# IBM/DeepRest

Measured on AMD Instinct MI355X. Metric: training samples/sec, 256-endpoint 3-resource estimation model, higher is better.
Workload: dtype bf16; 1 GPU; model=deeprest-amd (attention encoder + call-graph + GRU decoders), endpoints=256, components=63, num_metrics=192, global_batch=2048, seq_len=60, parallelism=dp1

## Files before the change

deeprest_amd/csrc/bindings.cpp:

```cpp
#include <torch/extension.h>
#include <ATen/cuda/CUDAContext.h>
#include <c10/cuda/CUDAGuard.h>
#include <hip/hip_runtime.h>

#include <cmath>
#include <string>
#include <vector>

extern "C" {
void dr_dropout_add_ln_fwd(const void* branch, const void* residual, const float* w,
                           const float* b, const int64_t* seed, uint32_t thr,
                           float scale, void* r_out, void* normed, float* mean,
                           float* rstd, int64_t n_rows, int D, float eps,
                           int is_bf16, hipStream_t stream);
void dr_dropout_add_ln_bwd(const void* d_normed, const void* d_r_out,
                           const void* r_out, const float* w, const float* mean,
                           const float* rstd, const int64_t* seed, uint32_t thr,
                           float scale, void* d_res, void* d_branch,
                           float* dwdb_part, int n_blocks, int64_t n_rows, int D,
                           int is_bf16, hipStream_t stream);
void dr_pinball_fwd(const void* out, const float* labels, const float* quantiles,
                    int Q, int64_t N, float inv_count, float* loss, int is_bf16,
                    hipStream_t stream);
void dr_pinball_bwd(const void* out, const float* labels, const float* quantiles,
// ... 4 lines not shown
                           const float* quantiles, int Q, int64_t R, int M,
                           float* wsum, int* wcnt, float* loss, float* w,
                           int is_bf16, hipStream_t stream);
void dr_pinball_masked_bwd(const void* out, const float* labels,
                           const float* quantiles, int Q, int64_t R, int M,
                           const float* grad_loss, const float* w, void* dout,
                           int is_bf16, hipStream_t stream);
void dr_fused_adam(const int64_t* meta, int nt, int64_t total, float lr, float beta1,
                   float beta2, float eps, float weight_decay, int step,
                   hipStream_t stream);
void dr_fused_adam_dev(const int64_t* meta, int nt, int64_t total,
                       const float* lr_ptr, float beta1, float beta2, float eps,
                       float weight_decay, const int* step_ptr,
                       hipStream_t stream);
int dr_gru_fwd_fuses_heads(int B, int C);
int dr_gru_fwd(const void* xg, const void* gamma, const void* beta,
               const void* w_hh, const float* b_hh, const void* h0, void* h_all,
               void* saves, const void* wh_fwd, void* out, int O, int B, int TT,
               int C, int reverse, int save, int fp8, int is_bf16,
               hipStream_t stream);
int dr_gru_decode(const void* xg, const void* gamma, const void* beta,
                  const void* w_hh, const float* b_hh, const void* h0,
                  const void* wh_fwd, void* out, void* h_last, int B, int TT,
                  int C, int O, int reverse, int fp8, int is_bf16,
                  const int* lens, hipStream_t stream);
int dr_gru_bwd(const void* grad, const void* wh_img, int O, const void* w_img,
               const void* w_fwd, const void* xg, const void* gamma,
               const void* beta, const float* b_hh, const void* h0,
               const void* h_all, const void* saves, void* dpre, float* dh0,
               int B, int TT, int C, int reverse, int is_bf16,
               hipStream_t stream);
int dr_gru_reduce_fused_max_c();
int dr_gru_bwd_reduce(const void* dpre, const void* gamma, const void* xg,
                      void* dxg, float* dgamma, float* dbeta, void* gamma_pi,
                      void* xg_pi, int64_t BT, int C, int mode, int is_bf16,
                      hipStream_t stream);
void dr_mha_fwd(const void* q, const void* k, const void* v, void* o, float* lse,
                int64_t BH, int T_len, int D, float scale, int is_bf16,
                const int* kv_len, int n_heads, hipStream_t stream);
void dr_mha_bwd(const void* q, const void* k, const void* v, const void* o,
                const void* dout, const float* lse, float* dq, void* dk, void* dv,
                int64_t BH, int T_len, int D, float scale, int is_bf16,
                hipStream_t stream);
int dr_sanity_scores(const void* out, const float* measured, const float* base,
                     const float* y_min, const float* y_scale,
// ... 349 lines not shown
              "gru operand dtypes must match x_gates");
  TORCH_CHECK(xg.is_contiguous() && w_hh.is_contiguous() && h0.is_contiguous() &&
              gamma.is_contiguous() && beta.is_contiguous() && b_hh.is_contiguous());
  TORCH_CHECK(xg.numel() < (1LL << 31),
              "x_gates too large for 32-bit staging offsets");
}

static void check_wh_fwd(const at::Tensor& wh_fwd, int64_t O, int H) {
  TORCH_CHECK(O >= 1 && O <= 32, "the fused head phase needs 1 <= O <= 32, got ", O);
  TORCH_CHECK(wh_fwd.scalar_type() == at::kBFloat16 &&
                  wh_fwd.sizes() == at::IntArrayRef({32, H}) &&
                  wh_fwd.is_contiguous() && wh_fwd.is_cuda(),
              "wh_fwd must be the (32, H) bf16 head weight image");
}

bool gru_fwd_fuses_heads(int64_t B, int64_t C, bool save) {
  return save && dr_gru_fwd_fuses_heads((int)B, (int)C) != 0;
}

std::vector<at::Tensor> gru_seq_forward(at::Tensor xg, at::Tensor w_hh,
                                        at::Tensor b_hh, at::Tensor h0,
                                        at::Tensor gamma, at::Tensor beta,
                                        bool reverse, bool save, bool fp8,
                                        c10::optional<at::Tensor> wh_fwd,
                                        int64_t O) {
  TORCH_CHECK(!(fp8 && save), "fp8 GRU path is inference-only (no saves)");
  const at::cuda::CUDAGuard guard(xg.device());
  gru_forward_checks(xg, w_hh, b_hh, h0, gamma, beta);
  int B = (int)xg.size(0), TT = (int)xg.size(1);
  int C = (int)h0.size(1), H = (int)h0.size(2);
// ... 2 lines not shown
  const bool heads = wh_fwd.has_value();
  if (heads) {
    TORCH_CHECK(!fp8 && gru_fwd_fuses_heads(B, C, save),
                "gru forward: no in-kernel head phase at B=", B, " C=", C,
                " save=", save, " (ask gru_fwd_fuses_heads first)");
    check_wh_fwd(*wh_fwd, O, H);
    TORCH_CHECK((int64_t)B * TT * C * O < (1LL << 31),
                "head output too large for 32-bit store offsets");
  }
  auto h_all = at::empty({B, TT, C, H}, xg.options());
  auto saves = save ? at::empty({B, TT, C, 2 * H}, xg.options())
                    : at::empty({0}, xg.options());
  auto out = heads ? at::empty({B, TT, C, O}, xg.options())
                   : at::empty({0}, xg.options());
  auto w_gemm = gru_w_gemm(w_hh);
  gru_launch_check(
      dr_gru_fwd(xg.data_ptr(), gamma.data_ptr(), beta.data_ptr(),
                 w_gemm.data_ptr(), b_hh.data_ptr<float>(), h0.data_ptr(),
                 h_all.data_ptr(), save ? saves.data_ptr() : nullptr,
                 heads ? wh_fwd->data_ptr() : nullptr,
                 heads ? out.data_ptr() : nullptr, heads ? (int)O : 0, B, TT, C,
                 reverse ? 1 : 0, save ? 1 : 0, fp8 ? 1 : 0, is_bf16(xg),
                 cur_stream()),
      "gru forward");
  if (!heads) return {h_all, saves};
  return {h_all, saves, out};
}

std::vector<at::Tensor> gru_seq_decode(at::Tensor xg, at::Tensor w_hh,
                                       at::Tensor b_hh, at::Tensor h0,
                                       at::Tensor gamma, at::Tensor beta,
                                       at::Tensor wh_fwd, int64_t O, bool reverse,
                                       bool fp8,
                                       c10::optional<at::Tensor> lengths) {
  const at::cuda::CUDAGuard guard(xg.device());
  gru_forward_checks(xg, w_hh, b_hh, h0, gamma, beta);
  int B = (int)xg.size(0), TT = (int)xg.size(1);
  int C = (int)h0.size(1), H = (int)h0.size(2);
  check_wh_fwd(wh_fwd, O, H);
  TORCH_CHECK((int64_t)B * TT * C * O < (1LL << 31),
              "decode output too large for 32-bit store offsets");
  const int* lens = lengths_ptr(lengths, xg, B, "gru decode lengths");
  auto out = lens ? at::zeros({B, TT, C, O}, xg.options())
                  : at::empty({B, TT, C, O}, xg.options());
  auto h_last = at::empty({B, C, H}, xg.options());
  auto w_gemm = gru_w_gemm(w_hh);
  gru_launch_check(
      dr_gru_decode(xg.data_ptr(), gamma.data_ptr(), beta.data_ptr(),
                    w_gemm.data_ptr(), b_hh.data_ptr<float>(), h0.data_ptr(),
                    wh_fwd.data_ptr(), out.data_ptr(), h_last.data_ptr(), B, TT,
                    C, (int)O, reverse ? 1 : 0, fp8 ? 1 : 0, is_bf16(xg), lens,
                    cur_stream()),
      "gru decode");
  return {out, h_last};
}

static std::vector<at::Tensor> gru_backward_impl(
    at::Tensor grad_h, const at::Tensor* wh_img, at::Tensor w_img,
    at::Tensor w_fwd, at::Tensor xg, at::Tensor gamma, at::Tensor beta,
    at::Tensor b_hh, at::Tensor h0, at::Tensor h_all, at::Tensor saves,
    bool reverse) {
  const at::cuda::CUDAGuard guard(grad_h.device());
  TORCH_CHECK(grad_h.dim() == 4 && h_all.dim() == 4, "grad and h_all must be 4-D");
  int B = (int)h_all.size(0), TT = (int)h_all.size(1);
  int C = (int)h_all.size(2), H = (int)h_all.size(3);
  TORCH_CHECK(H == 128);
  TORCH_CHECK(grad_h.size(0) == B && grad_h.size(1) == TT && grad_h.size(2) == C,
// ... 26 lines not shown
  TORCH_CHECK(w_img.scalar_type() == at::kBFloat16 &&
                  w_img.sizes() == at::IntArrayRef({H, 3 * H}) &&
                  w_img.is_contiguous(),
              "w_img must be the (H, 3H) bf16 pi-permuted W image");
  TORCH_CHECK(w_fwd.scalar_type() == at::kBFloat16 &&
                  w_fwd.sizes() == at::IntArrayRef({3 * H, H}) &&
                  w_fwd.is_contiguous(),
              "w_fwd must be the (3H, H) bf16 weight image");
  TORCH_CHECK(b_hh.scalar_type() == at::kFloat && b_hh.is_contiguous());
  auto dt = grad_h.scalar_type();
  TORCH_CHECK(xg.scalar_type() == dt && gamma.scalar_type() == dt &&
              beta.scalar_type() == dt);
  TORCH_CHECK(grad_h.is_contiguous() && h_all.is_contiguous() && saves.is_contiguous());
  auto dpre = at::empty({B, TT, C, 4 * H}, grad_h.options());
  auto dh0 = at::empty({B, C, H}, grad_h.options().dtype(at::kFloat));
  gru_launch_check(
      dr_gru_bwd(grad_h.data_ptr(), wh_img ? wh_img->data_ptr() : nullptr, O,
                 w_img.data_ptr(), w_fwd.data_ptr(), xg.data_ptr(),
                 gamma.data_ptr(), beta.data_ptr(), b_hh.data_ptr<float>(),
                 h0.data_ptr(), h_all.data_ptr(), saves.data_ptr(),
                 dpre.data_ptr(), dh0.data_ptr<float>(), B, TT, C,
                 reverse ? 1 : 0, dt == at::kBFloat16, cur_stream()),
      "gru backward");
  return {dpre, dh0};
}

std::vector<at::Tensor> gru_seq_backward_kernel(at::Tensor grad_h, at::Tensor w_img,
                                                at::Tensor w_fwd, at::Tensor xg,
                                                at::Tensor gamma, at::Tensor beta,
                                                at::Tensor b_hh, at::Tensor h0,
                                                at::Tensor h_all, at::Tensor saves,
                                                bool reverse) {
  return gru_backward_impl(grad_h, nullptr, w_img, w_fwd, xg, gamma, beta, b_hh,
                           h0, h_all, saves, reverse);
}

std::vector<at::Tensor> gru_seq_backward_heads_kernel(
// ... 198 lines not shown
```

deeprest_amd/csrc/common.h:

```cpp
#pragma once

#include <hip/hip_runtime.h>
#include <hip/hip_bf16.h>
#include <hip/hip_fp8.h>
#include <stdint.h>
#include <algorithm>

#define DR_WAVE 64

namespace dr {

__device__ __forceinline__ float bf2f(uint16_t x) {
  union { uint32_t u; float f; } v;
  v.u = static_cast<uint32_t>(x) << 16;
  return v.f;
}

__device__ __forceinline__ uint16_t f2bf(float f) {
  __hip_bfloat16 b = __float2bfloat16(f);
  return *reinterpret_cast<uint16_t*>(&b);
}

__device__ __forceinline__ uint32_t f2bf2(float lo, float hi) {
  __hip_bfloat162 b2 = __float22bfloat162_rn(make_float2(lo, hi));
// ... 42 lines not shown
}

__device__ __forceinline__ float group16_sum(float v) {
#pragma unroll
  for (int off = 8; off > 0; off >>= 1) v += __shfl_xor(v, off, DR_WAVE);
  return v;
}

__device__ __forceinline__ float group16_max(float v) {
#pragma unroll
  for (int off = 8; off > 0; off >>= 1) v = fmaxf(v, __shfl_xor(v, off, DR_WAVE));
  return v;
}

__device__ __forceinline__ float sigmoidf_(float x) {
  return __fdividef(1.0f, 1.0f + __expf(-x));
}

__device__ __forceinline__ float tanhf_(float x) {
  float xc = fminf(fmaxf(x, -15.f), 15.f);
  float e = __expf(2.f * xc);
  return __fdividef(e - 1.f, e + 1.f);
}

using f32x4 = __attribute__((__vector_size__(4 * sizeof(float)))) float;
using bf16x8 = __attribute__((ext_vector_type(8))) __bf16;
using s16x8 = __attribute__((ext_vector_type(8))) short;

}
```

deeprest_amd/csrc/gru.hip:

```cpp
#include "common.h"

#include <type_traits>

namespace dr {

constexpr int H = 128;
constexpr int G3H = 384;
constexpr int G4H = 512;
constexpr int ROWS = 64;
constexpr int WAVES = 4;
constexpr int THREADS = WAVES * DR_WAVE;
constexpr int KT = H / 32;
constexpr int NT = G3H / 16;
constexpr int XG_SLOTS = 32;

constexpr int LDS_MAX = 163840;

template <bool FP8, int NSUB, bool HEADS>
struct FwdLds {
  static constexpr int ELT = FP8 ? 1 : 2;
  static constexpr int W = 0;
  static constexpr int WH = W + G3H * H * ELT;
  static constexpr int HM = WH + (HEADS ? 32 * H * 2 : 0);
  static constexpr int XG = HM + ROWS * NSUB * H * ELT;
// ... 62 lines not shown
template <typename T>
__device__ __forceinline__ void ld8(const T* src, float* v);
template <>
__device__ __forceinline__ void ld8<uint16_t>(const uint16_t* src, float* v) {
  uint4 raw = *reinterpret_cast<const uint4*>(src);
  const uint16_t* p = reinterpret_cast<const uint16_t*>(&raw);
#pragma unroll
  for (int e = 0; e < 8; ++e) v[e] = bf2f(p[e]);
}
template <>
__device__ __forceinline__ void ld8<float>(const float* src, float* v) {
  *reinterpret_cast<float4*>(v) = *reinterpret_cast<const float4*>(src);
  *reinterpret_cast<float4*>(v + 4) = *reinterpret_cast<const float4*>(src + 4);
}

template <typename T>
__device__ __forceinline__ void st_frag(T* dst, bf16x8 v);
template <>
__device__ __forceinline__ void st_frag<uint16_t>(uint16_t* dst, bf16x8 v) {
  *reinterpret_cast<uint4*>(dst) = *reinterpret_cast<const uint4*>(&v);
}
template <>
__device__ __forceinline__ void st_frag<float>(float* dst, bf16x8 v) {
  const uint16_t* p = reinterpret_cast<const uint16_t*>(&v);
#pragma unroll
  for (int e = 0; e < 8; ++e) dst[e] = bf2f(p[e]);
}

template <typename T>
__device__ __forceinline__ void ld_raw8(const T* src, uint16_t* out);
// ... 9 lines not shown
}

template <typename T>
__device__ __forceinline__ bf16x8 ld_frag(const T* src);
template <>
__device__ __forceinline__ bf16x8 ld_frag<uint16_t>(const uint16_t* src) {
  return *reinterpret_cast<const bf16x8*>(src);
}
template <>
__device__ __forceinline__ bf16x8 ld_frag<float>(const float* src) {
  uint16_t p[8];
#pragma unroll
  for (int e = 0; e < 8; ++e) p[e] = f2bf(src[e]);
  return *reinterpret_cast<bf16x8*>(p);
}

template <typename T, bool SAVE, bool FP8 = false, int NSUB = 1, bool HEADS = false,
          bool VARLEN = false>
__global__ __launch_bounds__(THREADS * NSUB) void gru_fwd_kernel(
    const T* __restrict__ xg,
    const T* __restrict__ gamma,
    const T* __restrict__ beta,
    const uint16_t* __restrict__ w_gemm,
    const float* __restrict__ b_hh,
    const T* __restrict__ h0,
    T* __restrict__ h_all,
    T* __restrict__ saves,
    int B, int TT, int C, int reverse,
    const uint16_t* __restrict__ wh_fwd,
    T* __restrict__ out,
    T* __restrict__ h_last,
    int O,
    const int* __restrict__ lens) {
  static_assert(HEADS || !VARLEN, "per-row lengths exist in the decode kernel only");
  static_assert(!(SAVE && (VARLEN || FP8)),
                "the saving kernels run full windows on bf16 GEMM tiles");
  extern __shared__ __attribute__((aligned(16))) char smem[];
  using L = FwdLds<FP8, NSUB, HEADS>;
  constexpr int BROWS = ROWS * NSUB;
  constexpr int BTHREADS = THREADS * NSUB;
  char* Wl = smem + L::W;
  char* WHl = smem + L::WH;
  char* Hl = smem + L::HM;
  char* XGl = smem + L::XG;
  constexpr bool GB_REGS = (NSUB == 1) && !(VARLEN && FP8);

  const int tid = threadIdx.x;
  const int wv = tid / DR_WAVE;
  const int lane = tid % DR_WAVE;
  const int64_t R = (int64_t)B * C;
  const int64_t r0 = (int64_t)blockIdx.x * BROWS;

  for (int id = tid; id < G3H * (H / 8); id += BTHREADS) {
    int j = id / (H / 8);
    int blk = id % (H / 8);
    bf16x8 v = *reinterpret_cast<const bf16x8*>(w_gemm + (int64_t)j * H + blk * 8);
    if constexpr (FP8) {
      const uint16_t* bv = reinterpret_cast<const uint16_t*>(&v);
      uint8_t q[8];
#pragma unroll
// ... 28 lines not shown
    b_of[i] = (int)(rr / C);
    comp_of[i] = (int)(rr % C);
  }
  int len_of[4];
  if constexpr (VARLEN) {
#pragma unroll
    for (int i = 0; i < 4; ++i) {
      len_of[i] = std::min(std::max(lens[b_of[i]], 1), TT);
    }
  }

  constexpr int GBN = GB_REGS ? 8 : 1;
  uint32_t gb[4][3][GBN];
  float bh[3][GBN];
  int gb_off[4];
#pragma unroll
  for (int i = 0; i < 4; ++i) gb_off[i] = comp_of[i] * G3H;
  if constexpr (GB_REGS) {
#pragma unroll
    for (int i = 0; i < 4; ++i) {
      const T* grow = gamma + gb_off[i];
      const T* brow = beta + gb_off[i];
#pragma unroll
      for (int g = 0; g < 3; ++g)
#pragma unroll
        for (int nt = 0; nt < 8; ++nt) {
          int col = g * H + nt * 16 + c_col;
          uint16_t gv = live[i] ? f2bf(ldf(grow + col)) : 0;
          uint16_t bv = live[i] ? f2bf(ldf(brow + col)) : 0;
          gb[i][g][nt] = ((uint32_t)bv << 16) | gv;
        }
    }
// ... 58 lines not shown
  const uint16_t* xg_rows[4];
#pragma unroll
  for (int i = 0; i < 4; ++i)
    xg_rows[i] =
        reinterpret_cast<const uint16_t*>(XGl) +
        (wv * WSLOTS + std::min(b_of[i] - b_wlo, WSLOTS - 1)) * G3H + c_col * 8;

  __syncthreads();

  int stage_toff = 0;
  int bc_toff = 0;
  const int stage_tstep = (reverse ? -1 : 1) * G3H;
  for (int step = 0; step < TT; ++step) {
    const int t_now = reverse ? (TT - 1 - step) : step;
    (void)t_now;
    bf16x8 afrag[KT];
    int64_t afrag8[KT];
#pragma unroll
    for (int kt = 0; kt < KT; ++kt) {
      if constexpr (FP8)
        afrag8[kt] = *reinterpret_cast<const int64_t*>(Hl + afrag_off[kt]);
      else
        afrag[kt] = lds_read8(Hl, afrag_off[kt]);
    }

#pragma unroll
    for (int u = 0; u < MAXCH; ++u) {
      if (u < n_stage) {
        const T* src = xg + stage_soff[u] + stage_toff;
        uint16_t* dst = reinterpret_cast<uint16_t*>(XGl) + stage_pi0[u];
// ... 12 lines not shown
#pragma unroll
      for (int kt = 0; kt < KT; ++kt) {
        int j = nt * 16 + c_col;
        int k0 = kt * 32 + (lane >> 4) * 8;
        if constexpr (FP8) {
          int64_t bfrag = *reinterpret_cast<const int64_t*>(Wl + swz8(j, k0));
          a = __builtin_amdgcn_mfma_f32_16x16x32_fp8_fp8(afrag8[kt], bfrag, a, 0, 0, 0);
        } else {
          bf16x8 bfrag = lds_read8(Wl, swz(j, k0));
          a = __builtin_amdgcn_mfma_f32_16x16x32_bf16(afrag[kt], bfrag, a, 0, 0, 0);
        }
      }
      acc[nt] = a;
    }

    const T* gm_v = gamma;
    const T* bt_v = beta;
    const float* bh_v = b_hh;
    if constexpr (!GB_REGS) asm volatile("" : "+v"(gm_v), "+v"(bt_v), "+v"(bh_v));
#pragma unroll
    for (int i = 0; i < 4; ++i) {
      const T* grow = gm_v + gb_off[i];
      const T* brow = bt_v + gb_off[i];
      float fr[8], fz[8], fn[8];
      bool active = true;
      if constexpr (VARLEN) active = t_now < len_of[i];
#pragma unroll
      for (int nt = 0; nt < 8; ++nt) {
        float xr = bf2f(xg_rows[i][nt]);
        float xz = bf2f(xg_rows[i][H + nt]);
        float xn = bf2f(xg_rows[i][2 * H + nt]);
        int col = nt * 16 + c_col;
        float gmr, gmz, gmn, btr, btz, btn, bhr, bhz, bhn;
        if constexpr (GB_REGS) {
          gmr = bf2f((uint16_t)gb[i][0][nt]); btr = bf2f((uint16_t)(gb[i][0][nt] >> 16));
          gmz = bf2f((uint16_t)gb[i][1][nt]); btz = bf2f((uint16_t)(gb[i][1][nt] >> 16));
          gmn = bf2f((uint16_t)gb[i][2][nt]); btn = bf2f((uint16_t)(gb[i][2][nt] >> 16));
          bhr = bh[0][nt]; bhz = bh[1][nt]; bhn = bh[2][nt];
        } else if constexpr (NSUB == 1) {
          gmr = bf2f(f2bf(ldf(grow + col))); btr = bf2f(f2bf(ldf(brow + col)));
          gmz = bf2f(f2bf(ldf(grow + H + col)));
          btz = bf2f(f2bf(ldf(brow + H + col)));
          gmn = bf2f(f2bf(ldf(grow + 2 * H + col)));
          btn = bf2f(f2bf(ldf(brow + 2 * H + col)));
          bhr = bh_v[col]; bhz = bh_v[H + col]; bhn = bh_v[2 * H + col];
        } else {
          gmr = ldf(grow + col); btr = ldf(brow + col);
          gmz = ldf(grow + H + col); btz = ldf(brow + H + col);
          gmn = ldf(grow + 2 * H + col); btn = ldf(brow + 2 * H + col);
          bhr = bh_v[col]; bhz = bh_v[H + col]; bhn = bh_v[2 * H + col];
        }
        float g_r, g_z, g_n;
        if constexpr (!GB_REGS && NSUB == 1) {
          g_r = __fmul_rn(xr, gmr) + btr;
          g_z = __fmul_rn(xz, gmz) + btz;
          g_n = __builtin_fmaf(xn, gmn, btn);
        } else {
          g_r = xr * gmr + btr;
          g_z = xz * gmz + btz;
          g_n = xn * gmn + btn;
        }
        float rp = sigmoidf_(acc[nt][i] + bhr + g_r);
        float zp = sigmoidf_(acc[nt + 8][i] + bhz + g_z);
        float hn = acc[nt + 16][i] + bhn;
        float nn = tanhf_(g_n + rp * hn);
        float hnew = (1.f - zp) * nn + zp * h[i][nt];
        if constexpr (VARLEN) hnew = active ? hnew : h[i][nt];
        h[i][nt] = hnew;
        if constexpr (FP8)
          *reinterpret_cast<uint8_t*>(Hl + swz8(row_of[i], col)) = f2fp8(hnew);
        else
          *reinterpret_cast<uint16_t*>(Hl + swz(row_of[i], col)) = f2bf(hnew);
        fr[nt] = rp; fz[nt] = zp; fn[nt] = nn; (void)fn;
      }
      if (SAVE && live[i]) {
        T* sv = saves + (int64_t)(bc[i] + bc_toff) * (2 * H) + c_col * 8;
        st8(sv, fr);
        st8(sv + H, fz);
      }
      __builtin_amdgcn_sched_barrier(0);
    }
    wave_lds_fence();

    if constexpr (HEADS) {
      bf16x8 hfrag[KT];
#pragma unroll
      for (int kt = 0; kt < KT; ++kt) {
        if constexpr (FP8) {
          uint64_t raw = *reinterpret_cast<const uint64_t*>(Hl + afrag_off[kt]);
          const uint8_t* q = reinterpret_cast<const uint8_t*>(&raw);
          uint16_t p[8];
#pragma unroll
          for (int e = 0; e < 8; ++e) {
            __hip_fp8_e4m3 x;
            x.__x = q[e];
// ... 206 lines not shown
        const int jl = nt * 16 + c_col;
#pragma unroll
        for (int kt = 0; kt < KT; ++kt) {
          bf16x8 bfrag;
          if constexpr (NSUB == 2)
            bfrag = lds_read8(wn_lds, swz(jl, kt * 32 + k0));
          else
            bfrag = *reinterpret_cast<const bf16x8*>(
                wfv + (int64_t)(2 * H + jl) * H + kt * 32 + k0);
          a = __builtin_amdgcn_mfma_f32_16x16x32_bf16(hfrag[kt], bfrag, a, 0, 0, 0);
        }
        hhn_acc[nt] = a;
      }
    }

    const T* gm_v = gamma;
    const T* bt_v = beta;
    asm volatile("" : "+v"(gm_v), "+v"(bt_v));
#pragma unroll
    for (int i = 0; i < 4; ++i) {
      if (!live[i]) continue;
      const int64_t bc = bc0[i] + bc_toff;
      const T* sv_p = saves + bc * (2 * H) + c_col * 8;
      float rp[8], zp[8];
      ld8(sv_p, rp);
      ld8(sv_p + H, zp);
      float fdr[8], fdz[8], fdn[8], fdh[8];
      const T* hsrc = use_h0 ? (h0 + h0_off[i])
                             : (h_all + (bc + dirC) * H);
      const T* gr_p = grad_h + bc * H;
      const T* xg_n = xg + xgb0[i] + xg_toff + 2 * H;
      const T* gmn = gm_v + comp_of[i] * G3H + 2 * H;
      const T* btn = bt_v + comp_of[i] * G3H + 2 * H;
#pragma unroll
      for (int nt = 0; nt < 8; ++nt) {
        int col = nt * 16 + c_col;
        float hp = ldf(hsrc + col);
        float hn = hhn_acc[nt][i] + bhn[nt];
        float g_n = ldf(xg_n + col) * ldf(gmn + col) + ldf(btn + col);
        float nn = tanhf_(g_n + rp[nt] * hn);
        float dht = dh_carry[nt][i];
        if constexpr (!FUSED) dht += ldf(gr_p + col);
        float dz = dht * (hp - nn);
        float dn = dht * (1.f - zp[nt]);
        float dnp = dn * (1.f - nn * nn);
        float dhhn = dnp * rp[nt];
        float dr = dnp * hn;
        fdr[nt] = dr * rp[nt] * (1.f - rp[nt]);
        fdz[nt] = dz * zp[nt] * (1.f - zp[nt]);
        fdn[nt] = dnp;
        fdh[nt] = dhhn;
        dh_carry[nt][i] = dht * zp[nt];
      }
      T* dx_p = dpre + bc * G4H + c_col * 8;
// ... 54 lines not shown

template <typename T>
__global__ void pi_permute_rows_kernel(const T* __restrict__ in,
                                       T* __restrict__ out, int64_t N) {
  const int64_t n_chunks = N * 48;
  for (int64_t idx = (int64_t)blockIdx.x * blockDim.x + threadIdx.x;
       idx < n_chunks; idx += (int64_t)gridDim.x * blockDim.x) {
    const int64_t r = idx / 48;
    const int rem = (int)(idx % 48);
    const int g = rem / 16;
    const int cc = rem % 16;
    const T* src = in + r * G3H + g * H + cc;
    T* dst = out + r * G3H + g * H + cc * 8;
#pragma unroll
    for (int e = 0; e < 8; ++e) dst[e] = src[e * 16];
  }
}

template <typename T>
__global__ void gru_dxg_kernel(const T* __restrict__ dpre,
                               const T* __restrict__ gamma_pi,
                               T* __restrict__ dxg,
                               int64_t BT, int C) {
  const int64_t n_chunks = BT * 48;
  for (int64_t idx = (int64_t)blockIdx.x * blockDim.x + threadIdx.x; idx < n_chunks;
       idx += (int64_t)gridDim.x * blockDim.x) {
    const int64_t bt = idx / 48;
    const int rem = (int)(idx % 48);
    const int g = rem / 16;
    const int cc = rem % 16;
// ... 296 lines not shown
  const int64_t tiles128 = ((int64_t)B * C + 2 * ROWS - 1) / (2 * ROWS);
  const bool wide = !fp8 && tiles128 >= 192 && C >= 5;
  if (!wide && !fp8) return f(FwdTile<false, 1>{});
  if (fp8) return f(FwdTile<true, 1>{});
  return f(FwdTile<false, 2>{});
}
template <typename Tile>
static constexpr bool fwd_train_heads(Tile) { return !Tile::FP8 && Tile::NSUB == 2; }

template <typename K>
static hipError_t allow_lds(K kernel, int bytes) {
  return hipFuncSetAttribute(reinterpret_cast<const void*>(kernel),
                             hipFuncAttributeMaxDynamicSharedMemorySize, bytes);
}

struct FwdArgs {
  const void *xg, *gamma, *beta, *w_gemm;
  const float* b_hh;
  const void* h0;
  void *h_all, *saves;
  int B, TT, C, reverse;
  const void* wh_fwd;
  void *out, *h_last;
  int O;
  const int* lens;
  hipStream_t stream;
};

template <typename T, bool SAVE, bool FP8, int NSUB, bool HEADS, bool VARLEN>
static hipError_t gru_fwd_launch(const FwdArgs& a) {
  constexpr int LDS = FwdLds<FP8, NSUB, HEADS>::TOTAL;
  static const hipError_t attr =
      allow_lds(&gru_fwd_kernel<T, SAVE, FP8, NSUB, HEADS, VARLEN>, LDS);
  if (attr != hipSuccess) return attr;
  const int64_t R = (int64_t)a.B * a.C;
  const int grid = (int)((R + ROWS * NSUB - 1) / (ROWS * NSUB));
  hipLaunchKernelGGL((gru_fwd_kernel<T, SAVE, FP8, NSUB, HEADS, VARLEN>),
                     dim3(grid), dim3(THREADS * NSUB), LDS, a.stream,
                     (const T*)a.xg, (const T*)a.gamma, (const T*)a.beta,
                     (const uint16_t*)a.w_gemm, a.b_hh, (const T*)a.h0,
                     (T*)a.h_all, (T*)a.saves, a.B, a.TT, a.C, a.reverse,
                     (const uint16_t*)a.wh_fwd, (T*)a.out, (T*)a.h_last, a.O,
                     a.lens);
  return hipGetLastError();
}

struct BwdArgs {
  const void *grad, *wh_img, *w_img, *w_fwd, *xg, *gamma, *beta;
  const float* b_hh;
  const void *h0, *h_all, *saves;
  void* dpre;
  float* dh0;
  int B, TT, C, reverse, O;
  hipStream_t stream;
};

template <typename T, int NSUB, bool FUSED>
static hipError_t gru_bwd_launch(const BwdArgs& a) {
  constexpr int LDS = BwdLds<NSUB, FUSED>::TOTAL;
  static const hipError_t attr =
      LDS ? allow_lds(&gru_bwd_kernel<T, NSUB, FUSED>, LDS) : hipSuccess;
  if (attr != hipSuccess) return attr;
  const int64_t R = (int64_t)a.B * a.C;
  const int grid = (int)((R + ROWS * NSUB - 1) / (ROWS * NSUB));
  hipLaunchKernelGGL((gru_bwd_kernel<T, NSUB, FUSED>), dim3(grid),
                     dim3(THREADS * NSUB), LDS, a.stream, (const T*)a.grad,
                     (const uint16_t*)a.wh_img, (const uint16_t*)a.w_img,
                     (const uint16_t*)a.w_fwd, (const T*)a.xg,
                     (const T*)a.gamma, (const T*)a.beta, a.b_hh,
                     (const T*)a.h0, (const T*)a.h_all, (const T*)a.saves,
                     (T*)a.dpre, a.dh0, a.B, a.TT, a.C, a.reverse, a.O);
  return hipGetLastError();
}

static int cu_count() {
  int dev = 0, n = 0;
  if (hipGetDevice(&dev) != hipSuccess ||
      hipDeviceGetAttribute(&n, hipDeviceAttributeMultiprocessorCount, dev) != hipSuccess ||
      n <= 0)
    n = 256;
  return n;
}

template <typename T, int CPT>
// ... 47 lines not shown
  }
  hipLaunchKernelGGL((gru_dxg_kernel<T>), dim3(chunk_grid(BT)), dim3(256), 0,
                     stream, (const T*)dpre, (const T*)gamma_pi, (T*)dxg, BT, C);
  if (hipError_t e = hipGetLastError()) return e;
  const int gx = (C * 64 + 255) / 256;
  const int gy = 128;
  hipLaunchKernelGGL((gru_dgamma_kernel<T>), dim3(gx, gy), dim3(256), 0, stream,
                     (const T*)dpre, (const T*)xg_pi, dgamma, dbeta, BT, C);
  return hipGetLastError();
}

}

extern "C" {

int dr_gru_fwd_fuses_heads(int B, int C) {
  bool fuses = false;
  (void)dr::with_fwd_tile(B, C, 0, [&](auto tile) {
    fuses = dr::fwd_train_heads(tile);
    return hipSuccess;
  });
  return fuses ? 1 : 0;
}

int dr_gru_fwd(const void* xg, const void* gamma, const void* beta,
               const void* w_hh, const float* b_hh, const void* h0, void* h_all,
               void* saves, const void* wh_fwd, void* out, int O, int B, int TT,
               int C, int reverse, int save, int fp8, int is_bf16,
               hipStream_t stream) {
  const bool heads = wh_fwd != nullptr;
  const dr::FwdArgs a{xg, gamma, beta, w_hh, b_hh, h0, h_all, saves, B, TT, C,
                      reverse, wh_fwd, out, nullptr, heads ? O : 0, nullptr, stream};
  if (heads && !save) return (int)hipErrorInvalidValue;
  return (int)dr::with_io_type(is_bf16, [&](auto io) {
    using T = typename decltype(io)::type;
    return dr::with_fwd_tile(B, C, fp8, [&](auto tile) {
      using V = decltype(tile);
      if constexpr (dr::fwd_train_heads(V{})) {
        if (heads) return dr::gru_fwd_launch<T, true, false, V::NSUB, true, false>(a);
      } else {
        if (heads) return hipErrorInvalidValue;
      }
      if constexpr (!V::FP8)
        if (save) return dr::gru_fwd_launch<T, true, false, V::NSUB, false, false>(a);
      return dr::gru_fwd_launch<T, false, V::FP8, V::NSUB, false, false>(a);
    });
  });
}

int dr_gru_decode(const void* xg, const void* gamma, const void* beta,
                  const void* w_hh, const float* b_hh, const void* h0,
                  const void* wh_fwd, void* out, void* h_last, int B, int TT,
                  int C, int O, int reverse, int fp8, int is_bf16,
                  const int* lens, hipStream_t stream) {
  const dr::FwdArgs a{xg, gamma, beta, w_hh, b_hh, h0, nullptr, nullptr, B, TT, C,
                      reverse, wh_fwd, out, h_last, O, lens, stream};
  auto run = [&](auto varlen) {
    return dr::with_io_type(is_bf16, [&](auto io) {
      using T = typename decltype(io)::type;
      return dr::with_fwd_tile(B, C, fp8, [&](auto tile) {
        using V = decltype(tile);
        return dr::gru_fwd_launch<T, false, V::FP8, V::NSUB, true,
                                  decltype(varlen)::value>(a);
      });
    });
  };
  return (int)(lens != nullptr ? run(std::true_type{}) : run(std::false_type{}));
}

int dr_gru_bwd(const void* grad, const void* wh_img, int O, const void* w_img,
               const void* w_fwd, const void* xg, const void* gamma,
               const void* beta, const float* b_hh, const void* h0,
               const void* h_all, const void* saves, void* dpre, float* dh0,
               int B, int TT, int C, int reverse, int is_bf16,
               hipStream_t stream) {
  const bool fused = wh_img != nullptr;
  const dr::BwdArgs a{grad, wh_img, w_img, w_fwd, xg, gamma, beta, b_hh, h0,
                      h_all, saves, dpre, dh0, B, TT, C, reverse, fused ? O : 0,
                      stream};
  const int64_t tiles128 = ((int64_t)B * C + 2 * dr::ROWS - 1) / (2 * dr::ROWS);
  const bool lds_w = tiles128 >= 192;
  auto run = [&](auto fused_tag) {
    return dr::with_io_type(is_bf16, [&](auto io) {
      using T = typename decltype(io)::type;
      constexpr bool FUSED = decltype(fused_tag)::value;
      return lds_w ? dr::gru_bwd_launch<T, 2, FUSED>(a)
                   : dr::gru_bwd_launch<T, 1, FUSED>(a);
    });
  };
  return (int)(fused ? run(std::true_type{}) : run(std::false_type{}));
}

int dr_gru_reduce_fused_max_c() { return dr::REDUCE_FUSED_MAX_C; }

// ... 13 lines not shown
```

Baseline: 59510 windows/s.

## Pre-permute GRU gamma/beta/b_hh images for vectorized per-step loads

Adds a small pre-kernel that rewrites the FiLM gamma, beta and b_hh vectors into a per-lane contiguous layout. The GRU forward (non-register path) and backward kernels can then fetch eight values with one wide load instead of strided scalar loads on every timestep. The forward gate loop is restructured into a 12-stage software pipeline that issues the next stage's loads ahead of use. Sigmoid and tanh now use the hardware reciprocal instead of a division. The cost is an extra kernel launch and a scratch allocation per GRU call, plus small numeric differences from the reciprocal.

```diff
diff --git a/deeprest_amd/csrc/bindings.cpp b/deeprest_amd/csrc/bindings.cpp
--- a/deeprest_amd/csrc/bindings.cpp
+++ b/deeprest_amd/csrc/bindings.cpp
@@ -42,21 +42,22 @@
                        float weight_decay, const int* step_ptr,
                        hipStream_t stream);
 int dr_gru_fwd_fuses_heads(int B, int C);
+int64_t dr_gru_operand_images_bytes(int C, int is_bf16);
 int dr_gru_fwd(const void* xg, const void* gamma, const void* beta,
                const void* w_hh, const float* b_hh, const void* h0, void* h_all,
                void* saves, const void* wh_fwd, void* out, int O, int B, int TT,
-               int C, int reverse, int save, int fp8, int is_bf16,
+               int C, int reverse, int save, int fp8, int is_bf16, void* images,
                hipStream_t stream);
 int dr_gru_decode(const void* xg, const void* gamma, const void* beta,
                   const void* w_hh, const float* b_hh, const void* h0,
                   const void* wh_fwd, void* out, void* h_last, int B, int TT,
                   int C, int O, int reverse, int fp8, int is_bf16,
-                  const int* lens, hipStream_t stream);
+                  const int* lens, void* images, hipStream_t stream);
 int dr_gru_bwd(const void* grad, const void* wh_img, int O, const void* w_img,
                const void* w_fwd, const void* xg, const void* gamma,
                const void* beta, const float* b_hh, const void* h0,
                const void* h_all, const void* saves, void* dpre, float* dh0,
-               int B, int TT, int C, int reverse, int is_bf16,
+               int B, int TT, int C, int reverse, int is_bf16, void* images,
                hipStream_t stream);
 int dr_gru_reduce_fused_max_c();
 int dr_gru_bwd_reduce(const void* dpre, const void* gamma, const void* xg,
@@ -436,6 +437,11 @@
               "wh_fwd must be the (32, H) bf16 head weight image");
 }
 
+static at::Tensor gru_operand_images(const at::Tensor& gamma, int C) {
+  return at::empty({dr_gru_operand_images_bytes(C, is_bf16(gamma))},
+                   gamma.options().dtype(at::kByte));
+}
+
 bool gru_fwd_fuses_heads(int64_t B, int64_t C, bool save) {
   return save && dr_gru_fwd_fuses_heads((int)B, (int)C) != 0;
 }
@@ -468,6 +474,7 @@
   auto out = heads ? at::empty({B, TT, C, O}, xg.options())
                    : at::empty({0}, xg.options());
   auto w_gemm = gru_w_gemm(w_hh);
+  auto images = gru_operand_images(gamma, C);
   gru_launch_check(
       dr_gru_fwd(xg.data_ptr(), gamma.data_ptr(), beta.data_ptr(),
                  w_gemm.data_ptr(), b_hh.data_ptr<float>(), h0.data_ptr(),
@@ -475,7 +482,7 @@
                  heads ? wh_fwd->data_ptr() : nullptr,
                  heads ? out.data_ptr() : nullptr, heads ? (int)O : 0, B, TT, C,
                  reverse ? 1 : 0, save ? 1 : 0, fp8 ? 1 : 0, is_bf16(xg),
-                 cur_stream()),
+                 images.data_ptr(), cur_stream()),
       "gru forward");
   if (!heads) return {h_all, saves};
   return {h_all, saves, out};
@@ -499,12 +506,13 @@
                   : at::empty({B, TT, C, O}, xg.options());
   auto h_last = at::empty({B, C, H}, xg.options());
   auto w_gemm = gru_w_gemm(w_hh);
+  auto images = gru_operand_images(gamma, C);
   gru_launch_check(
       dr_gru_decode(xg.data_ptr(), gamma.data_ptr(), beta.data_ptr(),
                     w_gemm.data_ptr(), b_hh.data_ptr<float>(), h0.data_ptr(),
                     wh_fwd.data_ptr(), out.data_ptr(), h_last.data_ptr(), B, TT,
                     C, (int)O, reverse ? 1 : 0, fp8 ? 1 : 0, is_bf16(xg), lens,
-                    cur_stream()),
+                    images.data_ptr(), cur_stream()),
       "gru decode");
   return {out, h_last};
 }
@@ -561,13 +569,15 @@
   TORCH_CHECK(grad_h.is_contiguous() && h_all.is_contiguous() && saves.is_contiguous());
   auto dpre = at::empty({B, TT, C, 4 * H}, grad_h.options());
   auto dh0 = at::empty({B, C, H}, grad_h.options().dtype(at::kFloat));
+  auto images = gru_operand_images(gamma, C);
   gru_launch_check(
       dr_gru_bwd(grad_h.data_ptr(), wh_img ? wh_img->data_ptr() : nullptr, O,
                  w_img.data_ptr(), w_fwd.data_ptr(), xg.data_ptr(),
                  gamma.data_ptr(), beta.data_ptr(), b_hh.data_ptr<float>(),
                  h0.data_ptr(), h_all.data_ptr(), saves.data_ptr(),
                  dpre.data_ptr(), dh0.data_ptr<float>(), B, TT, C,
-                 reverse ? 1 : 0, dt == at::kBFloat16, cur_stream()),
+                 reverse ? 1 : 0, dt == at::kBFloat16, images.data_ptr(),
+                 cur_stream()),
       "gru backward");
   return {dpre, dh0};
 }
diff --git a/deeprest_amd/csrc/common.h b/deeprest_amd/csrc/common.h
--- a/deeprest_amd/csrc/common.h
+++ b/deeprest_amd/csrc/common.h
@@ -80,13 +80,13 @@
 }
 
 __device__ __forceinline__ float sigmoidf_(float x) {
-  return __fdividef(1.0f, 1.0f + __expf(-x));
+  return __builtin_amdgcn_rcpf(1.0f + __expf(-x));
 }
 
 __device__ __forceinline__ float tanhf_(float x) {
   float xc = fminf(fmaxf(x, -15.f), 15.f);
   float e = __expf(2.f * xc);
-  return __fdividef(e - 1.f, e + 1.f);
+  return (e - 1.f) * __builtin_amdgcn_rcpf(e + 1.f);
 }
 
 using f32x4 = __attribute__((__vector_size__(4 * sizeof(float)))) float;
diff --git a/deeprest_amd/csrc/gru.hip b/deeprest_amd/csrc/gru.hip
--- a/deeprest_amd/csrc/gru.hip
+++ b/deeprest_amd/csrc/gru.hip
@@ -100,6 +100,44 @@
   *reinterpret_cast<float4*>(v + 4) = *reinterpret_cast<const float4*>(src + 4);
 }
 
+template <typename T> struct Raw8;
+template <> struct Raw8<uint16_t> { uint4 v; };
+template <> struct Raw8<float> { float4 a, b; };
+__device__ __forceinline__ void widen8(const Raw8<uint16_t>& p, float* v) {
+  const uint32_t w[4] = {p.v.x, p.v.y, p.v.z, p.v.w};
+#pragma unroll
+  for (int i = 0; i < 4; ++i) {
+    v[2 * i] = __uint_as_float(w[i] << 16);
+    v[2 * i + 1] = __uint_as_float(w[i] & 0xffff0000u);
+  }
+}
+__device__ __forceinline__ void widen8(const Raw8<float>& p, float* v) {
+  v[0] = p.a.x; v[1] = p.a.y; v[2] = p.a.z; v[3] = p.a.w;
+  v[4] = p.b.x; v[5] = p.b.y; v[6] = p.b.z; v[7] = p.b.w;
+}
+template <typename T>
+__device__ __forceinline__ Raw8<T> ld_raw_at(const T* base, uint32_t byte_off);
+template <>
+__device__ __forceinline__ Raw8<uint16_t> ld_raw_at<uint16_t>(const uint16_t* base,
+                                                              uint32_t byte_off) {
+  return {*reinterpret_cast<const uint4*>(reinterpret_cast<const char*>(base) + byte_off)};
+}
+template <>
+__device__ __forceinline__ Raw8<float> ld_raw_at<float>(const float* base,
+                                                        uint32_t byte_off) {
+  const char* p = reinterpret_cast<const char*>(base) + byte_off;
+  return {*reinterpret_cast<const float4*>(p), *reinterpret_cast<const float4*>(p + 16)};
+}
+__device__ __forceinline__ float mul_rounded(float a, float b) {
+#pragma clang fp contract(off)
+  return a * b;
+}
+__device__ __forceinline__ uint32_t opaque_zero() {
+  uint32_t z = 0;
+  asm volatile("" : "+v"(z));
+  return z;
+}
+
 template <typename T>
 __device__ __forceinline__ void st_frag(T* dst, bf16x8 v);
 template <>
@@ -139,6 +177,9 @@
   for (int e = 0; e < 8; ++e) p[e] = f2bf(src[e]);
   return *reinterpret_cast<bf16x8*>(p);
 }
+
+template <bool FP8, int NSUB, bool VARLEN>
+constexpr bool fwd_gb_regs = (NSUB == 1) && !(VARLEN && FP8);
 
 template <typename T, bool SAVE, bool FP8 = false, int NSUB = 1, bool HEADS = false,
           bool VARLEN = false>
@@ -168,7 +209,7 @@
   char* WHl = smem + L::WH;
   char* Hl = smem + L::HM;
   char* XGl = smem + L::XG;
-  constexpr bool GB_REGS = (NSUB == 1) && !(VARLEN && FP8);
+  constexpr bool GB_REGS = fwd_gb_regs<FP8, NSUB, VARLEN>;
 
   const int tid = threadIdx.x;
   const int wv = tid / DR_WAVE;
@@ -227,8 +268,12 @@
   uint32_t gb[4][3][GBN];
   float bh[3][GBN];
   int gb_off[4];
-#pragma unroll
-  for (int i = 0; i < 4; ++i) gb_off[i] = comp_of[i] * G3H;
+  uint32_t gbi_off[4];
+#pragma unroll
+  for (int i = 0; i < 4; ++i) {
+    gb_off[i] = comp_of[i] * G3H;
+    gbi_off[i] = (uint32_t)(comp_of[i] * G3H + c_col * 8) * (uint32_t)sizeof(T);
+  }
   if constexpr (GB_REGS) {
 #pragma unroll
     for (int i = 0; i < 4; ++i) {
@@ -317,6 +362,9 @@
   for (int step = 0; step < TT; ++step) {
     const int t_now = reverse ? (TT - 1 - step) : step;
     (void)t_now;
+    uint32_t zoff = 0;
+    if constexpr (!GB_REGS) zoff = opaque_zero();
+    (void)zoff;
     bf16x8 afrag[KT];
     int64_t afrag8[KT];
 #pragma unroll
@@ -359,71 +407,132 @@
       acc[nt] = a;
     }
 
-    const T* gm_v = gamma;
-    const T* bt_v = beta;
-    const float* bh_v = b_hh;
-    if constexpr (!GB_REGS) asm volatile("" : "+v"(gm_v), "+v"(bt_v), "+v"(bh_v));
-#pragma unroll
-    for (int i = 0; i < 4; ++i) {
-      const T* grow = gm_v + gb_off[i];
-      const T* brow = bt_v + gb_off[i];
-      float fr[8], fz[8], fn[8];
-      bool active = true;
-      if constexpr (VARLEN) active = t_now < len_of[i];
-#pragma unroll
-      for (int nt = 0; nt < 8; ++nt) {
-        float xr = bf2f(xg_rows[i][nt]);
-        float xz = bf2f(xg_rows[i][H + nt]);
-        float xn = bf2f(xg_rows[i][2 * H + nt]);
-        int col = nt * 16 + c_col;
-        float gmr, gmz, gmn, btr, btz, btn, bhr, bhz, bhn;
-        if constexpr (GB_REGS) {
-          gmr = bf2f((uint16_t)gb[i][0][nt]); btr = bf2f((uint16_t)(gb[i][0][nt] >> 16));
-          gmz = bf2f((uint16_t)gb[i][1][nt]); btz = bf2f((uint16_t)(gb[i][1][nt] >> 16));
-          gmn = bf2f((uint16_t)gb[i][2][nt]); btn = bf2f((uint16_t)(gb[i][2][nt] >> 16));
-          bhr = bh[0][nt]; bhz = bh[1][nt]; bhn = bh[2][nt];
-        } else if constexpr (NSUB == 1) {
-          gmr = bf2f(f2bf(ldf(grow + col))); btr = bf2f(f2bf(ldf(brow + col)));
-          gmz = bf2f(f2bf(ldf(grow + H + col)));
-          btz = bf2f(f2bf(ldf(brow + H + col)));
-          gmn = bf2f(f2bf(ldf(grow + 2 * H + col)));
-          btn = bf2f(f2bf(ldf(brow + 2 * H + col)));
-          bhr = bh_v[col]; bhz = bh_v[H + col]; bhn = bh_v[2 * H + col];
+    if constexpr (GB_REGS) {
+#pragma unroll
+      for (int i = 0; i < 4; ++i) {
+        float fr[8], fz[8];
+        bool active = true;
+        if constexpr (VARLEN) active = t_now < len_of[i];
+#pragma unroll
+        for (int nt = 0; nt < 8; ++nt) {
+          float xr = bf2f(xg_rows[i][nt]);
+          float xz = bf2f(xg_rows[i][H + nt]);
+          float xn = bf2f(xg_rows[i][2 * H + nt]);
+          int col = nt * 16 + c_col;
+          float gmr = bf2f((uint16_t)gb[i][0][nt]), btr = bf2f((uint16_t)(gb[i][0][nt] >> 16));
+          float gmz = bf2f((uint16_t)gb[i][1][nt]), btz = bf2f((uint16_t)(gb[i][1][nt] >> 16));
+          float gmn = bf2f((uint16_t)gb[i][2][nt]), btn = bf2f((uint16_t)(gb[i][2][nt] >> 16));
+          float bhr = bh[0][nt], bhz = bh[1][nt], bhn = bh[2][nt];
+          float g_r = xr * gmr + btr;
+          float g_z = xz * gmz + btz;
+          float g_n = xn * gmn + btn;
+          float rp = sigmoidf_(acc[nt][i] + bhr + g_r);
+          float zp = sigmoidf_(acc[nt + 8][i] + bhz + g_z);
+          float hn = acc[nt + 16][i] + bhn;
+          float nn = tanhf_(g_n + rp * hn);
+          float hnew = (1.f - zp) * nn + zp * h[i][nt];
+          if constexpr (VARLEN) hnew = active ? hnew : h[i][nt];
+          h[i][nt] = hnew;
+          if constexpr (FP8)
+            *reinterpret_cast<uint8_t*>(Hl + swz8(row_of[i], col)) = f2fp8(hnew);
+          else
+            *reinterpret_cast<uint16_t*>(Hl + swz(row_of[i], col)) = f2bf(hnew);
+          fr[nt] = rp; fz[nt] = zp;
+        }
+        if (SAVE && live[i]) {
+          T* sv = saves + (int64_t)(bc[i] + bc_toff) * (2 * H) + c_col * 8;
+          st8(sv, fr);
+          st8(sv + H, fz);
+        }
+        __builtin_amdgcn_sched_barrier(0);
+      }
+    } else {
+      struct Stage { Raw8<T> gm, bt; };
+      auto issue = [&](int i, int g) {
+        const uint32_t off = gbi_off[i] + zoff + (uint32_t)(g * H * sizeof(T));
+        return Stage{ld_raw_at<T>(gamma, off), ld_raw_at<T>(beta, off)};
+      };
+      auto film = [&](const Stage& st, int i, int g, float* out) {
+        float xv[8], gmv[8], btv[8];
+        widen8(Raw8<uint16_t>{*reinterpret_cast<const uint4*>(xg_rows[i] + g * H)}, xv);
+        widen8(st.gm, gmv);
+        widen8(st.bt, btv);
+#pragma unroll
+        for (int nt = 0; nt < 8; ++nt) {
+          if constexpr (NSUB == 1) {
+            float gm = gmv[nt], bt = btv[nt];
+            if constexpr (sizeof(T) == 4) { gm = bf2f(f2bf(gm)); bt = bf2f(f2bf(bt)); }
+            out[nt] = g < 2 ? mul_rounded(xv[nt], gm) + bt : __builtin_fmaf(xv[nt], gm, bt);
+          } else {
+            out[nt] = __builtin_fmaf(xv[nt], gmv[nt], btv[nt]);
+          }
+        }
+      };
+#pragma unroll
+      for (int g = 0; g < 3; ++g) {
+        float bv[8];
+        widen8(ld_raw_at<float>(b_hh, (uint32_t)(g * H + c_col * 8) * 4u + zoff), bv);
+#pragma unroll
+        for (int nt = 0; nt < 8; ++nt)
+#pragma unroll
+          for (int i = 0; i < 4; ++i) acc[g * 8 + nt][i] += bv[nt];
+      }
+      constexpr int MIRROR_ROW_SHIFT = FP8 ? 3 : 4;
+      constexpr int MIRROR_NT_SHIFT = MIRROR_ROW_SHIFT + 1;
+      constexpr int MIRROR_ROW_BYTES = FP8 ? 128 : 256;
+      const int hm0 = (FP8 ? swz8(row_of[0], c_col) : swz(row_of[0], c_col)) + (int)zoff;
+      constexpr bool AHEAD = sizeof(T) == 2;
+      Stage cur, nxt;
+      if constexpr (AHEAD) cur = issue(0, 0);
+      __builtin_amdgcn_sched_barrier(0);
+      float fr[8], fz[8];
+#pragma unroll
+      for (int s = 0; s < 12; ++s) {
+        const int i = s / 3, g = s % 3;
+        if constexpr (AHEAD) {
+          if (s + 1 < 12) nxt = issue((s + 1) / 3, (s + 1) % 3);
         } else {
-          gmr = ldf(grow + col); btr = ldf(brow + col);
-          gmz = ldf(grow + H + col); btz = ldf(brow + H + col);
-          gmn = ldf(grow + 2 * H + col); btn = ldf(brow + 2 * H + col);
-          bhr = bh_v[col]; bhz = bh_v[H + col]; bhn = bh_v[2 * H + col];
+          cur = issue(i, g);
         }
-        float g_r, g_z, g_n;
-        if constexpr (!GB_REGS && NSUB == 1) {
-          g_r = __fmul_rn(xr, gmr) + btr;
-          g_z = __fmul_rn(xz, gmz) + btz;
-          g_n = __builtin_fmaf(xn, gmn, btn);
+        float pre[8];
+        film(cur, i, g, pre);
+        if (g == 0) {
+#pragma unroll
+          for (int nt = 0; nt < 8; ++nt) fr[nt] = sigmoidf_(acc[nt][i] + pre[nt]);
+        } else if (g == 1) {
+#pragma unroll
+          for (int nt = 0; nt < 8; ++nt) fz[nt] = sigmoidf_(acc[nt + 8][i] + pre[nt]);
         } else {
-          g_r = xr * gmr + btr;
-          g_z = xz * gmz + btz;
-          g_n = xn * gmn + btn;
+          bool active = true;
+          if constexpr (VARLEN) active = t_now < len_of[i];
+#pragma unroll
+          for (int nt = 0; nt < 8; ++nt) {
+            const float hn = acc[nt + 16][i];
+            const float rp = fr[nt], zp = fz[nt];
+            float nn = tanhf_(pre[nt] + rp * hn);
+            float hnew;
+            if constexpr (NSUB == 1)
+              hnew = mul_rounded(1.f - zp, nn) + mul_rounded(zp, h[i][nt]);
+            else
+              hnew = __builtin_fmaf(zp, h[i][nt], mul_rounded(1.f - zp, nn));
+            if constexpr (VARLEN) hnew = active ? hnew : h[i][nt];
+            h[i][nt] = hnew;
+            char* hm_p = Hl + (hm0 ^ ((i << MIRROR_ROW_SHIFT) ^ (nt << MIRROR_NT_SHIFT))) +
+                         i * MIRROR_ROW_BYTES;
+            if constexpr (FP8)
+              *reinterpret_cast<uint8_t*>(hm_p) = f2fp8(hnew);
+            else
+              *reinterpret_cast<uint16_t*>(hm_p) = f2bf(hnew);
+          }
+          if (SAVE && live[i]) {
+            T* sv = saves + (int64_t)(bc[i] + bc_toff) * (2 * H) + c_col * 8;
+            st8(sv, fr);
+            st8(sv + H, fz);
+          }
         }
-        float rp = sigmoidf_(acc[nt][i] + bhr + g_r);
-        float zp = sigmoidf_(acc[nt + 8][i] + bhz + g_z);
-        float hn = acc[nt + 16][i] + bhn;
-        float nn = tanhf_(g_n + rp * hn);
-        float hnew = (1.f - zp) * nn + zp * h[i][nt];
-        if constexpr (VARLEN) hnew = active ? hnew : h[i][nt];
-        h[i][nt] = hnew;
-        if constexpr (FP8)
-          *reinterpret_cast<uint8_t*>(Hl + swz8(row_of[i], col)) = f2fp8(hnew);
-        else
-          *reinterpret_cast<uint16_t*>(Hl + swz(row_of[i], col)) = f2bf(hnew);
-        fr[nt] = rp; fz[nt] = zp; fn[nt] = nn; (void)fn;
+        if constexpr (AHEAD) cur = nxt;
+        __builtin_amdgcn_sched_barrier(0);
       }
-      if (SAVE && live[i]) {
-        T* sv = saves + (int64_t)(bc[i] + bc_toff) * (2 * H) + c_col * 8;
-        st8(sv, fr);
-        st8(sv + H, fz);
-      }
-      __builtin_amdgcn_sched_barrier(0);
     }
     wave_lds_fence();
 
@@ -660,9 +769,7 @@
       }
     }
 
-    const T* gm_v = gamma;
-    const T* bt_v = beta;
-    asm volatile("" : "+v"(gm_v), "+v"(bt_v));
+    const uint32_t zoff = opaque_zero();
 #pragma unroll
     for (int i = 0; i < 4; ++i) {
       if (!live[i]) continue;
@@ -676,14 +783,21 @@
                              : (h_all + (bc + dirC) * H);
       const T* gr_p = grad_h + bc * H;
       const T* xg_n = xg + xgb0[i] + xg_toff + 2 * H;
-      const T* gmn = gm_v + comp_of[i] * G3H + 2 * H;
-      const T* btn = bt_v + comp_of[i] * G3H + 2 * H;
+      float gmn[8], btn[8];
+      {
+        const uint32_t off =
+            (uint32_t)(comp_of[i] * G3H + 2 * H + c_col * 8) * (uint32_t)sizeof(T) + zoff;
+        const Raw8<T> gq = ld_raw_at<T>(gamma, off);
+        const Raw8<T> bq = ld_raw_at<T>(beta, off);
+        widen8(gq, gmn);
+        widen8(bq, btn);
+      }
 #pragma unroll
       for (int nt = 0; nt < 8; ++nt) {
         int col = nt * 16 + c_col;
         float hp = ldf(hsrc + col);
         float hn = hhn_acc[nt][i] + bhn[nt];
-        float g_n = ldf(xg_n + col) * ldf(gmn + col) + ldf(btn + col);
+        float g_n = ldf(xg_n + col) * gmn[nt] + btn[nt];
         float nn = tanhf_(g_n + rp[nt] * hn);
         float dht = dh_carry[nt][i];
         if constexpr (!FUSED) dht += ldf(gr_p + col);
@@ -768,6 +882,38 @@
     T* dst = out + r * G3H + g * H + cc * 8;
 #pragma unroll
     for (int e = 0; e < 8; ++e) dst[e] = src[e * 16];
+  }
+}
+
+template <typename T>
+struct OperandImages {
+  static int64_t gamma(int C) { (void)C; return 0; }
+  static int64_t beta(int C) { return (int64_t)C * G3H * (int64_t)sizeof(T); }
+  static int64_t bhh(int C) { return 2 * beta(C); }
+  static int64_t total(int C) { return bhh(C) + G3H * 4; }
+};
+
+template <typename T>
+__global__ void gru_operand_images_kernel(const T* __restrict__ gamma,
+                                          const T* __restrict__ beta,
+                                          const float* __restrict__ b_hh,
+                                          T* __restrict__ gamma_pi,
+                                          T* __restrict__ beta_pi,
+                                          float* __restrict__ bhh_pi, int C) {
+  const int idx = blockIdx.x * blockDim.x + threadIdx.x;
+  if (idx >= (2 * C + 1) * 48) return;
+  const int r = idx / 48;
+  const int rem = idx % 48;
+  const int src = (rem / 16) * H + rem % 16;
+  const int dst = (rem / 16) * H + (rem % 16) * 8;
+  if (r < 2 * C) {
+    const T* in = (r < C ? gamma + r * G3H : beta + (r - C) * G3H) + src;
+    T* out = (r < C ? gamma_pi + r * G3H : beta_pi + (r - C) * G3H) + dst;
+#pragma unroll
+    for (int e = 0; e < 8; ++e) out[e] = in[e * 16];
+  } else {
+#pragma unroll
+    for (int e = 0; e < 8; ++e) bhh_pi[dst + e] = b_hh[src + e * 16];
   }
 }
 
@@ -1094,6 +1240,21 @@
                              hipFuncAttributeMaxDynamicSharedMemorySize, bytes);
 }
 
+template <typename T>
+static hipError_t operand_images_launch(const void* gamma, const void* beta,
+                                        const float* b_hh, void* images, int C,
+                                        hipStream_t stream) {
+  if (images == nullptr) return hipErrorInvalidValue;
+  using I = OperandImages<T>;
+  char* img = static_cast<char*>(images);
+  const int n = (2 * C + 1) * 48;
+  hipLaunchKernelGGL((gru_operand_images_kernel<T>), dim3((n + 255) / 256), dim3(256),
+                     0, stream, (const T*)gamma, (const T*)beta, b_hh,
+                     (T*)(img + I::gamma(C)), (T*)(img + I::beta(C)),
+                     (float*)(img + I::bhh(C)), C);
+  return hipGetLastError();
+}
+
 struct FwdArgs {
   const void *xg, *gamma, *beta, *w_gemm;
   const float* b_hh;
@@ -1104,6 +1265,7 @@
   void *out, *h_last;
   int O;
   const int* lens;
+  void* images;
   hipStream_t stream;
 };
 
@@ -1115,10 +1277,22 @@
   if (attr != hipSuccess) return attr;
   const int64_t R = (int64_t)a.B * a.C;
   const int grid = (int)((R + ROWS * NSUB - 1) / (ROWS * NSUB));
+  const void *gamma = a.gamma, *beta = a.beta;
+  const float* b_hh = a.b_hh;
+  if constexpr (!fwd_gb_regs<FP8, NSUB, VARLEN>) {
+    if (hipError_t e = operand_images_launch<T>(a.gamma, a.beta, a.b_hh, a.images,
+                                                a.C, a.stream))
+      return e;
+    using I = OperandImages<T>;
+    const char* img = static_cast<const char*>(a.images);
+    gamma = img + I::gamma(a.C);
+    beta = img + I::beta(a.C);
+    b_hh = reinterpret_cast<const float*>(img + I::bhh(a.C));
+  }
   hipLaunchKernelGGL((gru_fwd_kernel<T, SAVE, FP8, NSUB, HEADS, VARLEN>),
                      dim3(grid), dim3(THREADS * NSUB), LDS, a.stream,
-                     (const T*)a.xg, (const T*)a.gamma, (const T*)a.beta,
-                     (const uint16_t*)a.w_gemm, a.b_hh, (const T*)a.h0,
+                     (const T*)a.xg, (const T*)gamma, (const T*)beta,
+                     (const uint16_t*)a.w_gemm, b_hh, (const T*)a.h0,
                      (T*)a.h_all, (T*)a.saves, a.B, a.TT, a.C, a.reverse,
                      (const uint16_t*)a.wh_fwd, (T*)a.out, (T*)a.h_last, a.O,
                      a.lens);
@@ -1132,6 +1306,7 @@
   void* dpre;
   float* dh0;
   int B, TT, C, reverse, O;
+  void* images;
   hipStream_t stream;
 };
 
@@ -1143,11 +1318,17 @@
   if (attr != hipSuccess) return attr;
   const int64_t R = (int64_t)a.B * a.C;
   const int grid = (int)((R + ROWS * NSUB - 1) / (ROWS * NSUB));
+  if (hipError_t e = operand_images_launch<T>(a.gamma, a.beta, a.b_hh, a.images,
+                                              a.C, a.stream))
+    return e;
+  using I = OperandImages<T>;
+  const char* img = static_cast<const char*>(a.images);
   hipLaunchKernelGGL((gru_bwd_kernel<T, NSUB, FUSED>), dim3(grid),
                      dim3(THREADS * NSUB), LDS, a.stream, (const T*)a.grad,
                      (const uint16_t*)a.wh_img, (const uint16_t*)a.w_img,
                      (const uint16_t*)a.w_fwd, (const T*)a.xg,
-                     (const T*)a.gamma, (const T*)a.beta, a.b_hh,
+                     (const T*)(img + I::gamma(a.C)), (const T*)(img + I::beta(a.C)),
+                     a.b_hh,
                      (const T*)a.h0, (const T*)a.h_all, (const T*)a.saves,
                      (T*)a.dpre, a.dh0, a.B, a.TT, a.C, a.reverse, a.O);
   return hipGetLastError();
@@ -1225,6 +1406,11 @@
 
 extern "C" {
 
+int64_t dr_gru_operand_images_bytes(int C, int is_bf16) {
+  return is_bf16 ? dr::OperandImages<uint16_t>::total(C)
+                 : dr::OperandImages<float>::total(C);
+}
+
 int dr_gru_fwd_fuses_heads(int B, int C) {
   bool fuses = false;
   (void)dr::with_fwd_tile(B, C, 0, [&](auto tile) {
@@ -1238,10 +1424,11 @@
                const void* w_hh, const float* b_hh, const void* h0, void* h_all,
                void* saves, const void* wh_fwd, void* out, int O, int B, int TT,
                int C, int reverse, int save, int fp8, int is_bf16,
-               hipStream_t stream) {
+               void* images, hipStream_t stream) {
   const bool heads = wh_fwd != nullptr;
   const dr::FwdArgs a{xg, gamma, beta, w_hh, b_hh, h0, h_all, saves, B, TT, C,
-                      reverse, wh_fwd, out, nullptr, heads ? O : 0, nullptr, stream};
+                      reverse, wh_fwd, out, nullptr, heads ? O : 0, nullptr, images,
+                      stream};
   if (heads && !save) return (int)hipErrorInvalidValue;
   return (int)dr::with_io_type(is_bf16, [&](auto io) {
     using T = typename decltype(io)::type;
@@ -1263,9 +1450,9 @@
                   const void* w_hh, const float* b_hh, const void* h0,
                   const void* wh_fwd, void* out, void* h_last, int B, int TT,
                   int C, int O, int reverse, int fp8, int is_bf16,
-                  const int* lens, hipStream_t stream) {
+                  const int* lens, void* images, hipStream_t stream) {
   const dr::FwdArgs a{xg, gamma, beta, w_hh, b_hh, h0, nullptr, nullptr, B, TT, C,
-                      reverse, wh_fwd, out, h_last, O, lens, stream};
+                      reverse, wh_fwd, out, h_last, O, lens, images, stream};
   auto run = [&](auto varlen) {
     return dr::with_io_type(is_bf16, [&](auto io) {
       using T = typename decltype(io)::type;
@@ -1283,12 +1470,12 @@
                const void* w_fwd, const void* xg, const void* gamma,
                const void* beta, const float* b_hh, const void* h0,
                const void* h_all, const void* saves, void* dpre, float* dh0,
-               int B, int TT, int C, int reverse, int is_bf16,
+               int B, int TT, int C, int reverse, int is_bf16, void* images,
                hipStream_t stream) {
   const bool fused = wh_img != nullptr;
   const dr::BwdArgs a{grad, wh_img, w_img, w_fwd, xg, gamma, beta, b_hh, h0,
                       h_all, saves, dpre, dh0, B, TT, C, reverse, fused ? O : 0,
-                      stream};
+                      images, stream};
   const int64_t tiles128 = ((int64_t)B * C + 2 * dr::ROWS - 1) / (2 * dr::ROWS);
   const bool lds_w = tiles128 >= 192;
   auto run = [&](auto fused_tag) {
```

New measurement: 65050 windows/s (median of 6 runs). 1.09x the previous value.
